# bing164/PL-VI-ORBSLAM3

Measured on AMD Instinct MI355X. Metric: frames/sec ORB+LSD extract+match, 640×480 mono, 1/2/4/8 MI355X, higher is better.
Workload: dtype u8; 1 GPU; C1+C2+C3: ORB extract (1000 feats, 1.2, 8 levels, FAST 20/7) || LSD+LBD (200 lines, scale 0.8, 2 octaves) as one HIP-stream schedule, then ORB kNN-2 + LineMatcher::match vs previous frame; batch=3072, width=640, height=480, parallelism=sequence-sharded x1, gather=False, inflight=2

## Files before the change

pl-vi-orbslam3_amd/csrc/lines_kernels.hpp:

```cpp
#include <hip/hip_runtime.h>

#include "block_prims.h"
#include "lines_device.h"
#include "plvi_common.h"
#include "plvi_math.h"
#include "std_sort.h"

namespace plvi {

constexpr double kNotdef = -1024.0;
constexpr float kNotdefF = -1024.0f;
constexpr double kD2R = 3.14159265358979323846 / 180;
constexpr double kPi = 3.14159265358979323846;
constexpr double kLog10Of11 = 0x1.0a98b6050c56fp+0;

__global__ __launch_bounds__(256) void lsd_half_kernel(const uint8_t* __restrict__ src, size_t s_frame, size_t s_row,
                                                       uint8_t* __restrict__ dst, int dw, int dh, size_t d_frame) {
    const int f = blockIdx.y;
    const int i = blockIdx.x * 256 + threadIdx.x;
    if (i >= dw * dh) return;
    const int y = i / dw, x = i % dw;
    const uint8_t* S0 = src + (size_t)f * s_frame + (size_t)(2 * y) * s_row;
    const uint8_t* S1 = S0 + s_row;
    const int s = S0[2 * x] + S0[2 * x + 1] + S1[2 * x] + S1[2 * x + 1];
// ... 1113 lines not shown
        const int D0 = sd - su, D1 = sd1 - su1;
        const int pk = S1 | (D1 + 1024) << 12, pkl = S0 | (D0 + 1024) << 12;
        const int L = dpp_from_left(pk);
        const int R = dpp_from_right(pkl);
        const int Sl = xl ? S1 : (L & 4095), Dl = xl ? D1 : (L >> 12) - 1024;
        const int Sr = xr ? S0 : (R & 4095), Dr = xr ? D0 : (R >> 12) - 1024;
        const bool last0 = xa + 1 >= w;
        const int Sr0 = last0 ? Sl : S1, Dr0 = last0 ? Dl : D1;
        const int gx0 = Sr0 - Sl, gy0 = Dl + 2 * D0 + Dr0;
        const int gx1 = Sr - S0, gy1 = D0 + 2 * D1 + Dr;
        short2* o = Gp + (size_t)y * w + xa;
        if (out0) o[0] = make_short2((short)gx0, (short)gy0);
        if (out1) o[1] = make_short2((short)gx1, (short)gy1);
    };
    uint32_t pv[8];
#pragma unroll
    for (int k = 0; k < 8; ++k) pv[k] = load_row(k - 2);
    const int rend = 2 * h + 3;
    for (int rb = -2; rb < rend - 2; rb += 8) {
#pragma unroll
        for (int k = 0; k < 8; ++k) {
            const int r = rb + k;
            if (r > 2 * h) break;
            const uint32_t V = pv[k];
            if (r + 8 <= 2 * h) pv[k] = load_row(r + 8);
#pragma unroll
            for (int q = 0; q < 4; ++q) {
                pe[q] = pe[q + 1];
                po[q] = po[q + 1];
            }
            pe[4] = V & 0x00ff00ffu;
            po[4] = (V >> 8) & 0x00ff00ffu;
            if ((k & 1) || r < 2) continue;
            const int y = (r - 2) >> 1;
            const uint32_t Ve = pe[0] + pe[4] + 4 * (pe[1] + pe[3]) + 6 * pe[2];
            const uint32_t Vo = po[0] + po[4] + 4 * (po[1] + po[3]) + 6 * po[2];
            const uint32_t Vel = (uint32_t)dpp_from_left((int)Ve), Vol = (uint32_t)dpp_from_left((int)Vo);
            const uint32_t Ver = (uint32_t)dpp_from_right((int)Ve);
            const uint32_t s0 = (Vel >> 16) + 4 * (Vol >> 16) + 6 * (Ve & 0xffffu) + 4 * (Vo & 0xffffu) + (Ve >> 16);
            const uint32_t s1 = (Ve & 0xffffu) + 4 * (Vo & 0xffffu) + 6 * (Ve >> 16) + 4 * (Vo >> 16) + (Ver & 0xffffu);
            const int P = (int)((s0 + 128u) >> 8) | (int)((s1 + 128u) >> 8) << 8;
            if (y == 1) sobel_row(0, P, p0, P);
            else if (y >= 2) sobel_row(y - 1, pm1, p0, P);
            pm1 = p0;
            p0 = P;
        }
    }
    if (h >= 2) sobel_row(h - 1, pm1, p0, pm1);
    else sobel_row(0, p0, p0, p0);
}

__constant__ float c_gaussG[63];
__constant__ float c_gaussL[21];
__constant__ unsigned char c_comb[64];

__global__ __launch_bounds__(64) void lbd_describe_kernel(const LineOctDev* __restrict__ octs,
                                                          const short2* __restrict__ g_all,
                                                          const plvi_keyline* __restrict__ kls,
                                                          const int* __restrict__ counts, int fcap,
                                                          uint8_t* __restrict__ desc) {
    __shared__ float rq[8][64];
    __shared__ float bs[72];
    __shared__ float dv[72];
    const int li = blockIdx.x, f = blockIdx.y;
    if (li >= counts[f]) return;
    const plvi_keyline kl = kls[(size_t)f * fcap + li];
    const LineOctDev& od = octs[kl.octave];
    const short2* pg = g_all + od.loff + (size_t)f * od.lplane;
    const short realWidth = (short)od.lw;
    const short imageWidth = realWidth - 1;
    const short imageHeight = (short)(od.lh - 1);
    const short lengthOfLSP = (short)kl.numOfPixels;
    const short halfWidth = (lengthOfLSP - 1) / 2;
    const short halfHeight = (63 - 1) / 2;
    const float mX = (float)(0.5 * (double)(kl.sPointInOctaveX + kl.ePointInOctaveX));
    const float mY = (float)(0.5 * (double)(kl.sPointInOctaveY + kl.ePointInOctaveY));
    const float dL0 = plvi_cosf(kl.angle), dL1 = plvi_sinf(kl.angle);
    const float dO0 = -dL1, dO1 = dL0;
    const int h = threadIdx.x;
    float pL = 0, nL = 0, pO = 0, nO = 0;
    __shared__ int sidx[64][9];
    auto& sg = sidx;
    {
        float sX = -dL0 * halfWidth + dL1 * halfHeight + mX;
        float sY = -dL1 * halfWidth - dL0 * halfHeight + mY;
        for (int k = 0; k < h; ++k) {
            sX -= dL1;
            sY += dL0;
        }
        const int* pgi = reinterpret_cast<const int*>(pg);
        const int kk = h & 7, rr = h >> 3;
        for (int w0 = 0; w0 < lengthOfLSP; w0 += 8) {
#pragma unroll
            for (int k = 0; k < 8; ++k) {
                short t = (short)__builtin_roundf(sX);
                const short xc = (t < 0) ? 0 : (t > imageWidth) ? imageWidth : t;
                t = (short)__builtin_roundf(sY);
                const short yc = (t < 0) ? 0 : (t > imageHeight) ? imageHeight : t;
                sidx[h][k] = yc * realWidth + xc;
                sX += dL0;
                sY += dL1;
            }
            __builtin_amdgcn_wave_barrier();
            __builtin_amdgcn_fence(__ATOMIC_ACQ_REL, "wavefront");
            int gv[8];
            const bool okk = w0 + kk < lengthOfLSP;
#pragma unroll
            for (int i = 0; i < 8; ++i) {
                const int r = 8 * i + rr;
                gv[i] = (r < 63 && okk) ? pgi[sidx[r][kk]] : 0;
            }
#pragma unroll
            for (int i = 0; i < 8; ++i) sg[8 * i + rr][kk] = gv[i];
            __builtin_amdgcn_wave_barrier();
            __builtin_amdgcn_fence(__ATOMIC_ACQ_REL, "wavefront");
            if (h < 63) {
#pragma unroll
                for (int k = 0; k < 8; ++k) {
                    if (w0 + k >= lengthOfLSP) break;
                    const short2 g = __builtin_bit_cast(short2, sg[h][k]);
                    const short dx = g.x, dy = g.y;
                    const float gDL = dx * dL0 + dy * dL1;
                    const float gDO = dx * dO0 + dy * dO1;
                    if (gDL > 0) pL += gDL;
                    else nL -= gDL;
                    if (gDO > 0) pO += gDO;
                    else nO -= gDO;
                }
            }
            __builtin_amdgcn_wave_barrier();
            __builtin_amdgcn_fence(__ATOMIC_ACQ_REL, "wavefront");
        }
    }
    if (h < 63) {
        const float c = c_gaussG[h];
        const float pLr = c * pL, nLr = c * nL, pOr = c * pO, nOr = c * nO;
        rq[0][h] = pLr; rq[1][h] = nLr; rq[2][h] = pLr * pLr; rq[3][h] = nLr * nLr;
        rq[4][h] = pOr; rq[5][h] = nOr; rq[6][h] = pOr * pOr; rq[7][h] = nOr * nOr;
    }
    __syncthreads();
    for (int a = h; a < 72; a += 64) {
        const int b = a >> 3, q = a & 7;
        const bool sq = (q & 2) != 0;
        float acc = 0.f;
        const int r0 = max(0, 7 * (b - 1)), r1 = min(62, 7 * (b + 2) - 1);
        for (int r = r0; r <= r1; ++r) {
            const int j = r / 7, m = r - 7 * j;
            const float c = j == b ? c_gaussL[m + 7] : j == b + 1 ? c_gaussL[m + 14] : c_gaussL[m];
            const float x = rq[q][r];
            acc += sq ? c * c * x : c * x;
        }
        bs[a] = acc;
    }
    __syncthreads();
    if (h < 36) {
        const int b = h >> 2, k = h & 3;
        const int qs = (k < 2 ? 0 : 4) + (k & 1);
        const float invN = (b == 0 || b == 8) ? (float)(1.0 / (7 * 2.0)) : (float)(1.0 / (7 * 3.0));
        const float t = bs[8 * b + qs] * invN;
        dv[8 * b + k] = t;
        dv[8 * b + 4 + k] = __builtin_sqrtf(bs[8 * b + qs + 2] * invN - t * t);
    }
    __syncthreads();
    __shared__ float s_t[3];
    if (h == 0) {
        float tM = 0, tS = 0;
        for (int b = 0; b < 9; ++b) {
            const float* v = dv + 8 * b;
            tM += v[0] * v[0]; tM += v[1] * v[1]; tM += v[2] * v[2]; tM += v[3] * v[3];
            tS += v[4] * v[4]; tS += v[5] * v[5]; tS += v[6] * v[6]; tS += v[7] * v[7];
        }
        s_t[0] = 1 / __builtin_sqrtf(tM);
        s_t[1] = 1 / __builtin_sqrtf(tS);
    }
    __syncthreads();
    for (int i = h; i < 72; i += 64) {
        float v = dv[i] * ((i & 7) < 4 ? s_t[0] : s_t[1]);
        if ((double)v > 0.4) v = (float)0.4;
        dv[i] = v;
    }
    __syncthreads();
    if (h == 0) {
        float t = 0;
        for (int i = 0; i < 72; ++i) t += dv[i] * dv[i];
        s_t[2] = 1 / __builtin_sqrtf(t);
    }
    __syncthreads();
    for (int i = h; i < 72; i += 64) dv[i] = dv[i] * s_t[2];
    __syncthreads();
    if (h < 32) {
        const float* f1 = dv + 8 * c_comb[2 * h];
        const float* f2 = dv + 8 * c_comb[2 * h + 1];
        unsigned r = 0;
        for (int i = 0; i < 8; ++i)
            if (f1[i] > f2[i]) r += 1u << i;
        desc[((size_t)f * fcap + li) * 32 + h] = (uint8_t)r;
    }
}

}
```

pl-vi-orbslam3_amd/csrc/lines_pipeline.hip:

```cpp
#include <hip/hip_runtime.h>

#include <algorithm>
#include <cmath>
#include <cstdlib>
#include <cstring>
#include <memory>
#include <vector>

#include "lines_device.h"
#include "lines_kernels.hpp"
#include "lsd_grow_mw.hpp"
#include "plvi_common.h"

extern "C" int plvi_orb_internal_blur_event(plvi_orb_extractor* h, hipEvent_t ev);
extern "C" int plvi_orb_internal_stage_event(plvi_orb_extractor* h, int stage, hipEvent_t ev);

namespace plvi {

static inline int lround_h(float v) { return (int)lrintf(v); }
static inline int lround_h(double v) { return (int)lrint(v); }
static inline int lfloor_h(float v) { int i = (int)v; return i - (i > v); }

static double cv_exp64f(double x) {
    const double a0s = .9670371139572337719125840413672004409288e-2;
// ... 12 lines not shown
}

static void gauss_kernel_f64(int n, double sigma, double* k, bool cvExp) {
    const double scale2X = -0.125 / (sigma * sigma);
    const int n2 = (n - 1) / 2;
    std::vector<double> values(n2 + 1);
    double sum = 0;
    for (int i = 0, x = 1 - n; i < n2; ++i, x += 2) {
        const double a = (double)(x * x) * scale2X;
        double t = cvExp ? cv_exp64f(a) : std::exp(a);
        values[i] = t;
        sum += t;
    }
    sum *= 2;
    sum += 1.0;
    const double mul1 = 1.0 / sum;
    for (int i = 0; i < n2; ++i) k[i] = k[n - 1 - i] = values[i] * mul1;
    k[n2] = 1.0 * mul1;
}

struct LinePipeline {
    plvi_line_params prm{};
    int W = 0, H = 0, Bcap = 0, device = 0, nOct = 0, fcap = 0;
    hipStream_t stream = nullptr;
    hipStream_t aux[2] = {nullptr, nullptr};
    hipEvent_t evSobelGo = nullptr;
    hipEvent_t evFork = nullptr, evPrep = nullptr, evSobel = nullptr, evOrb = nullptr, evCrit = nullptr,
               evBlur = nullptr, evGate = nullptr, evGrow2 = nullptr, evPair = nullptr;
    bool growAfterBlur = true, sobelWithGrow = false, growSplit = false;
    int sobelGate = -1;
    bool sobelAfterGrow = false;
    hipStream_t critStream = nullptr;
    hipStream_t crit2 = nullptr;
    hipStream_t octStream = nullptr;
    int orbAfterPrep = 1;
    std::vector<LineOctDev> oct;
    std::vector<float> scaleF, invScaleF;
    double SCALE = 0.8, prec = 0, rho = 0, min_length = 0;
    double gk[7]{};
    int lbdTaps[3] = {14, 62, 104};
    DevBuf d_oct, d_tabs, octImg, pix, modg, seedcs, gbits, qspill, regs, regpts, rawLines, nlines, klTmp, klOut, fnOut, cntOut, descOut, lbdBlur,
        lbdG, err, staging, mwOwn, mwSlot, mwGrow, sortPos;
    size_t qspillFrame = 0, gbitsFrame = 0, lbdPlaneTotal = 0;
    int lastFrames = 0;
    static constexpr int kStages = 5, kRing = 512;
    bool prof = false;
    int profRuns = 0;
    std::vector<hipEvent_t> evs;

    static constexpr int kKRing = 4096;
    bool ktime = false;
    int kn = 0;
    std::vector<hipEvent_t> kev;
    std::vector<hipEvent_t> kevS[3];
    int knS[3] = {0, 0, 0};
    int ktiming(int on) {
        if (on && kev.empty()) {
            kev.resize(2 * kKRing);
            for (auto& e : kev) PLVI_CHECK(hipEventCreate(&e));
            for (auto& v : kevS) {
                v.resize(2 * kKRing);
                for (auto& e : v) PLVI_CHECK(hipEventCreate(&e));
            }
        }
        ktime = on != 0;
        if (on) kn = knS[0] = knS[1] = knS[2] = 0;
        return PLVI_OK;
    }
    void ktimeS(int k, int edge, hipStream_t st) {
        if (!ktime || knS[k] >= kKRing) return;
        (void)hipEventRecord(kevS[k][2 * knS[k] + edge], st);
        if (edge) ++knS[k];
    }
    int ktiming_read_kind(int kind, float* total_ms, int* launches) {
        if (kind == 0) return ktiming_read(total_ms, launches);
        if (kind < 1 || kind > 3) return PLVI_E_BADARG;
        const int k = kind - 1;
        float tot = 0.f;
        for (int i = 0; i < knS[k]; ++i) {
            PLVI_CHECK(hipEventSynchronize(kevS[k][2 * i + 1]));
            float t = 0.f;
            PLVI_CHECK(hipEventElapsedTime(&t, kevS[k][2 * i], kevS[k][2 * i + 1]));
            tot += t;
        }
        if (total_ms) *total_ms = tot;
        if (launches) *launches = knS[k];
        return PLVI_OK;
    }
    int ktiming_read(float* total_ms, int* launches) {
        float tot = 0.f;
        for (int i = 0; i < kn; ++i) {
            PLVI_CHECK(hipEventSynchronize(kev[2 * i + 1]));
            float t = 0.f;
            PLVI_CHECK(hipEventElapsedTime(&t, kev[2 * i], kev[2 * i + 1]));
            tot += t;
        }
        if (total_ms) *total_ms = tot;
        if (launches) *launches = kn;
        return PLVI_OK;
    }

    ~LinePipeline() {
        for (auto e : kev) (void)hipEventDestroy(e);
        for (auto& v : kevS)
            for (auto e : v) (void)hipEventDestroy(e);
        for (auto e : evs) (void)hipEventDestroy(e);
        for (auto e : {evFork, evPrep, evSobel, evOrb, evCrit, evBlur, evGate, evGrow2, evPair, evSobelGo})
            if (e) (void)hipEventDestroy(e);
        if (critStream) (void)hipStreamDestroy(critStream);
        if (crit2) (void)hipStreamDestroy(crit2);
        if (octStream) (void)hipStreamDestroy(octStream);
        for (auto a : aux)
            if (a) (void)hipStreamDestroy(a);
        if (stream) (void)hipStreamDestroy(stream);
    }

    int init(const plvi_line_params* p, int width, int height, int max_batch, int dev) {
        if (!p || width <= 0 || height <= 0 || max_batch <= 0) return PLVI_E_BADARG;
        if (p->refine != 0 || p->extractor != 0) return PLVI_E_BADARG;
        if (p->nlevels <= 0 || p->nlevels > kLineMaxOct || p->nfeatures < 0) return PLVI_E_BADARG;
        prm = *p;
        W = width; H = height; Bcap = max_batch; device = dev; nOct = p->nlevels;
        PLVI_CHECK(hipSetDevice(device));
        PLVI_CHECK(hipStreamCreateWithFlags(&stream, hipStreamNonBlocking));
        {
            int least = 0, greatest = 0;
            PLVI_CHECK(hipDeviceGetStreamPriorityRange(&least, &greatest));
            const char* e1 = getenv("PLVI_STREAM_PRIO");
            const bool prio = !e1 || atoi(e1) != 0;
// ... 100 lines not shown
                    yb[2 * dy + 1] = fy;
                }
                d.xmax = xmax;
                std::vector<int> strips;
                for (int X0 = 0; X0 < d.sw;) {
                    const int gx0 = xofs[X0];
                    int E = X0;
                    while (E < d.sw && xofs[E] + (E < xmax ? 1 : 0) - gx0 + 3 <= 60) ++E;
                    const int X1 = E == d.sw ? E : E - 1;
                    if (X1 <= X0) return PLVI_E_BADARG;
                    strips.insert(strips.end(), {X0, X1, gx0, E - X0});
                    X0 = X1;
                }
                for (int dy = 0; dy < d.sh; ++dy) {
                    const int r1 = yrow[2 * dy + 1], r0 = yrow[2 * dy];
                    if (r0 > r1 || r1 - r0 > 1 || (dy > 0 && r1 < yrow[2 * dy - 1])) return PLVI_E_BADARG;
                }
                d.nstrips = (int)strips.size() / 4;
                d.tabStrips = put(strips.data(), strips.size() * 4);
                for (int nb : {1, kPrepBands}) {
                    std::vector<int> bands;
                    for (int b = 0; b < nb; ++b) {
                        const int dyA = (int)((long long)d.sh * b / nb), dyB = (int)((long long)d.sh * (b + 1) / nb);
                        bands.insert(bands.end(), {dyA, dyB, dyA == 0 ? -3 : yrow[2 * dyA] - 3, 0});
                    }
                    (nb == 1 ? d.tabBands1 : d.tabBandsK) = put(bands.data(), bands.size() * 4);
                }
                d.tabXofs = put(xofs.data(), xofs.size() * 4);
                d.tabXa = put(xa.data(), xa.size() * 4);
                d.tabYrow = put(yrow.data(), yrow.size() * 4);
                d.tabYb = put(yb.data(), yb.size() * 4);
            }
            d.lw = l == 0 ? W : oct[l - 1].lw / 2;
            d.lh = l == 0 ? H : oct[l - 1].lh / 2;
            d.lplane = (long long)d.lw * d.lh;
            d.loff = (long long)lOff;
            lOff += (size_t)d.lplane * Bcap;
        }
        lbdPlaneTotal = lOff;
        qspillFrame = (maxSplane + 1) & ~size_t(1);
        for (auto& d : oct) gbitsFrame = std::max(gbitsFrame, (size_t)d.sh * (size_t)((d.sw + 31) / 32));
        if (d_oct.alloc(sizeof(LineOctDev) * nOct) || d_tabs.alloc(tabs.size())) return PLVI_E_HIP;
        PLVI_CHECK(hipMemcpy(d_oct.p, oct.data(), sizeof(LineOctDev) * nOct, hipMemcpyHostToDevice));
        PLVI_CHECK(hipMemcpy(d_tabs.p, tabs.data(), tabs.size(), hipMemcpyHostToDevice));
        {
            float gL[21], gG[63];
            double u = (7 * 3 - 1) / 2, sg = (7 * 2 + 1) / 2, inv = -1 / (2 * sg * sg);
            for (int i = 0; i < 21; ++i) { double dis = i - u; gL[i] = (float)std::exp(dis * dis * inv); }
            u = (9 * 7 - 1) / 2; sg = u; inv = -1 / (2 * sg * sg);
            for (int i = 0; i < 63; ++i) { double dis = i - u; gG[i] = (float)std::exp(dis * dis * inv); }
            static const unsigned char comb[64] = {0, 1, 0, 2, 0, 3, 0, 4, 0, 5, 0, 6, 1, 2, 1, 3, 1, 4, 1, 5, 1, 6,
                                                   2, 3, 2, 4, 2, 5, 2, 6, 2, 7, 2, 8, 3, 4, 3, 5, 3, 6, 3, 7, 3, 8,
                                                   4, 5, 4, 6, 4, 7, 4, 8, 5, 6, 5, 7, 5, 8, 6, 7, 6, 8, 7, 8};
            PLVI_CHECK(hipMemcpyToSymbol(HIP_SYMBOL(c_gaussL), gL, sizeof(gL)));
            PLVI_CHECK(hipMemcpyToSymbol(HIP_SYMBOL(c_gaussG), gG, sizeof(gG)));
            PLVI_CHECK(hipMemcpyToSymbol(HIP_SYMBOL(c_comb), comb, sizeof(comb)));
        }
        if (octImg.alloc(std::max<size_t>(imgOff, 16)) || pix.alloc(sizeof(float) * sOff) ||
            modg.alloc(sizeof(double) * sOff) || seedcs.alloc(sizeof(float2) * sOff) ||
            gbits.alloc(sizeof(unsigned) * gbitsFrame * nOct * Bcap) || qspill.alloc(sizeof(unsigned) * qspillFrame * nOct * Bcap) ||
            rawLines.alloc(sizeof(LsdLine) * (size_t)kLsdRawCap * nOct * Bcap) ||
            regs.alloc(sizeof(LsdRegion) * (size_t)kLsdRawCap * nOct * Bcap) ||
            regpts.alloc(sizeof(unsigned) * qspillFrame * nOct * Bcap) ||
            nlines.alloc(sizeof(int) * nOct * Bcap) || klTmp.alloc(sizeof(plvi_keyline) * (size_t)kKlCap * Bcap) ||
            sortPos.alloc(sizeof(unsigned short) * 2 * (size_t)kKlCap * Bcap) ||
            klOut.alloc(sizeof(plvi_keyline) * (size_t)fcap * Bcap) || fnOut.alloc(sizeof(double) * 3 * fcap * Bcap) ||
            cntOut.alloc(sizeof(int) * Bcap) || descOut.alloc((size_t)32 * fcap * Bcap) ||
            lbdBlur.alloc((size_t)W * H * Bcap) || lbdG.alloc(sizeof(short2) * lbdPlaneTotal) ||
            err.alloc(sizeof(int) * Bcap) || staging.alloc((size_t)W * H))
            return PLVI_E_HIP;
        PLVI_CHECK(hipMemset(err.p, 0, sizeof(int) * Bcap));
        size_t maxSw = 0;
        for (auto& d : oct) maxSw = std::max(maxSw, (size_t)d.sw);
        const size_t wprMax = (maxSw + 31) / 32;
        size_t budget = 6 * 1024;
        if (const char* e = getenv("PLVI_GROW_LDS")) budget = (size_t)atol(e);
        budget = std::min<size_t>(budget, 160 * 1024);
        growRB = 64;
        if (const char* e = getenv("PLVI_GROW_RB")) growRB = atoi(e);
        if (growRB < 2 || (growRB & (growRB - 1)) || growRB > 1024) return PLVI_E_BADARG;
        growQL = budget >= 32 * 1024 ? 1024 : 256;
        const size_t fixed = (size_t)growQL * sizeof(unsigned) + (size_t)growRB * wprMax * sizeof(unsigned);
        const size_t perRow = maxSw * sizeof(float);
        growR = 0;
        if (fixed + perRow * 2 <= budget) {
            growR = 2;
            while (growR * 2 <= 1024 && fixed + perRow * growR * 2 <= budget) growR *= 2;
        }
        if (const char* e = getenv("PLVI_GROW_RD")) growR = atoi(e);
        if (growR < 0 || (growR & (growR - 1)) || growR == 1 || growR > 1024) return PLVI_E_BADARG;
        growSmem = (fixed + perRow * growR + 15) & ~size_t(15);
        if (growSmem > 160 * 1024) return PLVI_E_BADARG;
        growWPW = (int)std::max<size_t>(1, std::min<size_t>(kGrowWaves, (160 * 1024) / growSmem));
        for (const void* k : {(const void*)lsd_grow_kernel<false, false>, (const void*)lsd_grow_kernel<true, false>,
                              (const void*)lsd_grow_kernel<false, true>, (const void*)lsd_grow_kernel<true, true>,
                              (const void*)lsd_grow_kernel<false, true, true>})
            PLVI_CHECK(hipFuncSetAttribute(k, hipFuncAttributeMaxDynamicSharedMemorySize, (int)(growSmem * growWPW)));
        mwMaxFrames = 256;
        if (const char* e = getenv("PLVI_GROW_MW")) mwMaxFrames = atoi(e);
        if (const char* e = getenv("PLVI_GROW_TPW")) growTPW = std::max(0, atoi(e));
        mwMaxFrames = std::min(mwMaxFrames, Bcap);
        if (mwMaxFrames > 0) {
            const size_t nwords = gbitsFrame;
            const size_t fixedMw = sizeof(MwCtl) + 8 * kMwLog +
                                   4 * (3 * nwords + (size_t)kMwWaves * kMwRB * wprMax + (size_t)kMwWaves * kMwGQ);
            const size_t ldsMax = 160 * 1024;
            mwSlots = fixedMw < ldsMax ? (int)std::min<size_t>(kMwMaxSlots, (ldsMax - fixedMw) / kMwSlotBytes) : 0;
// ... 117 lines not shown
                           (const float2*)seedcs.as<float2>(), gbits.as<unsigned>(), gbitsFrame,
                           qspill.as<unsigned>(), qspillFrame, prec, regs.as<LsdRegion>(), regpts.as<unsigned>(),
                           qspillFrame, nlines.as<int>(), err.as<int>(), growR, growRB, growQL, nOct, oBase, oCount,
                           growStats, nf, (int)growSmem, growWPW);
    }
    void launch_rect(int nf, int oBase, int oCount, hipStream_t st) {
        const int bx = nf <= 16 ? 8 : nf < kRectLargeNf ? kRectLaneBlocks : kRectLaneBlocksLarge;
        auto rectK = nf <= kRectSmallNf ? lsd_rect_lanes_kernel<kRectUSmall> : lsd_rect_lanes_kernel<kRectU>;
        ktimeS(2, 0, st);
        hipLaunchKernelGGL(rectK, dim3(bx, nf, oCount), dim3(256), 0, st, d_oct.as<LineOctDev>(),
                           (const double*)modg.as<double>(), (const LsdRegion*)regs.as<LsdRegion>(),
                           (const unsigned*)regpts.as<unsigned>(), qspillFrame, (const int*)nlines.as<int>(), prec,
                           SCALE, rawLines.as<LsdLine>(), oBase, nOct, qspill.as<double>(), qspillFrame / 2,
                           (int)(qspillFrame / 2));
        ktimeS(2, 1, st);
    }
    void launch_grow_assemble(int nf, hipStream_t st, bool grown = false, bool rect0 = false) {
        if (!grown) launch_grow(nf, 0, nOct, st);
        launch_rect(nf, 0, rect0 ? 1 : nOct, st);
        mark(3, st);
        hipLaunchKernelGGL(line_assemble_kernel, dim3(nf), dim3(256), 0, st, d_oct.as<LineOctDev>(), nOct,
                           (const LsdLine*)rawLines.as<LsdLine>(), (const int*)nlines.as<int>(), min_length,
                           prm.nfeatures, fcap, klOut.as<plvi_keyline>(), fnOut.as<double>(), cntOut.as<int>(),
                           klTmp.as<plvi_keyline>(), err.as<int>(), sortPos.as<unsigned short>());
        mark(4, st);
    }

    int launch_sobel(const uint8_t* d_frames, int nf, size_t frame_stride, size_t row_stride, hipStream_t st) {
        const LineOctDev& d0 = oct[0];
        {
            const int ns = (d0.lw + 4 * kLbOutLanes - 1) / (4 * kLbOutLanes);
            const int sw4 = ((d0.lw + ns - 1) / ns + 3) & ~3;
            ktimeS(0, 0, st);
            hipLaunchKernelGGL(lbd_sobel0_kernel, dim3((d0.lw + sw4 - 1) / sw4, nf, kLbBands), dim3(64), 0, st, d_frames,
                               frame_stride, row_stride, d0.lw, d0.lh, sw4, lbdBlur.as<uint8_t>(),
                               lbdG.as<short2>() + d0.loff, (size_t)d0.lplane, lbdTaps[0], lbdTaps[1], lbdTaps[2]);
            ktimeS(0, 1, st);
        }
        for (int l = 1; l < nOct; ++l) {
            const LineOctDev& d = oct[l];
            if (l > 1) return PLVI_E_BADARG;
            const int ns = (d.lw + 2 * kLb2OutLanes - 1) / (2 * kLb2OutLanes);
            const int sw2 = ((d.lw + ns - 1) / ns + 1) & ~1;
            ktimeS(1, 0, st);
            hipLaunchKernelGGL(lbd_sobel1_kernel, dim3((d.lw + sw2 - 1) / sw2, nf), dim3(64), 0, st,
                               (const uint8_t*)lbdBlur.as<uint8_t>(), d0.lw, d0.lh, (size_t)d0.lplane, d.lw, d.lh,
                               sw2, lbdG.as<short2>() + d.loff, (size_t)d.lplane);
            ktimeS(1, 1, st);
        }
        return PLVI_OK;
    }

    void launch_describe(int nf, hipStream_t st) {
        hipLaunchKernelGGL(lbd_describe_kernel, dim3(fcap, nf), dim3(64), 0, st, d_oct.as<LineOctDev>(),
                           (const short2*)lbdG.as<short2>(),
                           (const plvi_keyline*)klOut.as<plvi_keyline>(), (const int*)cntOut.as<int>(), fcap,
                           descOut.as<uint8_t>());
        mark(5, st);
    }

    int run(const uint8_t* d_frames, int nf, size_t frame_stride, size_t row_stride, hipStream_t st) {
        if (nf <= 0 || nf > Bcap) return PLVI_E_BADARG;
        if (!st) st = stream;
        lastFrames = nf;
        hipStreamCaptureStatus cs = hipStreamCaptureStatusNone;
        PLVI_CHECK(hipStreamIsCapturing(st, &cs));
        const bool fork = !prof && aux[1] && cs == hipStreamCaptureStatusNone;
        int rc = PLVI_OK;
        if (fork) {
            PLVI_CHECK(hipEventRecord(evFork, st));
            PLVI_CHECK(hipStreamWaitEvent(aux[1], evFork, 0));
            rc = launch_sobel(d_frames, nf, frame_stride, row_stride, aux[1]);
            PLVI_CHECK(hipEventRecord(evSobel, aux[1]));
        }
        mark(0, st);
        if (fork && nOct > 1 && nf <= mwMaxFrames) {
            launch_prep(d_frames, nf, frame_stride, row_stride, st, 0, 1);
            PLVI_CHECK(hipEventRecord(evPrep, st));
            PLVI_CHECK(hipStreamWaitEvent(aux[0], evPrep, 0));
            launch_prep(d_frames, nf, frame_stride, row_stride, aux[0], 1, nOct);
            launch_grow(nf, 1, nOct - 1, aux[0]);
            launch_rect(nf, 1, nOct - 1, aux[0]);
            PLVI_CHECK(hipEventRecord(evGrow2, aux[0]));
            launch_grow(nf, 0, 1, st);
            PLVI_CHECK(hipStreamWaitEvent(st, evGrow2, 0));
            launch_grow_assemble(nf, st, true, true);
        } else {
            launch_prep(d_frames, nf, frame_stride, row_stride, st);
            launch_grow_assemble(nf, st);
        }
        if (fork) {
            PLVI_CHECK(hipStreamWaitEvent(st, evSobel, 0));
        } else {
            rc = launch_sobel(d_frames, nf, frame_stride, row_stride, st);
        }
        if (rc) return rc;
        launch_describe(nf, st);
        if (prof && profRuns < kRing) ++profRuns;
        PLVI_CHECK(hipGetLastError());
        return PLVI_OK;
    }

    struct StepMatch {
        int *idx0, *d0, *idx1, *d1;
        float nnr;
        int *lscratch, *lm12, *lnm;
    };
    int run_with_orb(const uint8_t* d_frames, int nf, size_t frame_stride, size_t row_stride, hipStream_t st,
                     plvi_orb_extractor* orb, int lap0, int lap1, const StepMatch* sm = nullptr) {
        if (nf <= 0 || nf > Bcap) return PLVI_E_BADARG;
// ... 371 lines not shown
```

pl-vi-orbslam3_amd/csrc/plvi_math.h:

```cpp
#pragma once
#include <stdint.h>
#include <string.h>

#ifdef __HIPCC__
#define PLVI_HD __host__ __device__ __forceinline__
#else
#define PLVI_HD static inline
#endif

namespace plvi {

PLVI_HD uint32_t f2u(float f) { uint32_t u; memcpy(&u, &f, 4); return u; }
PLVI_HD float u2f(uint32_t u) { float f; memcpy(&f, &u, 4); return f; }
PLVI_HD uint64_t d2u(double d) { uint64_t u; memcpy(&u, &d, 8); return u; }
PLVI_HD double u2d(uint64_t u) { double d; memcpy(&d, &u, 8); return d; }
PLVI_HD double fmad(double a, double b, double c) { return __builtin_fma(a, b, c); }

PLVI_HD double rfma(double a, double b, double c) { return __builtin_fma(a, b, c); }
PLVI_HD float rfmaf(float a, float b, float c) { return __builtin_fmaf(a, b, c); }

struct SinCosF {
    double c0, c1, s1, c2, s2, c3, s3, c4;
};
#define PLVI_HPI_INV 0x1.45f306dc9c883p+23
// ... 72 lines not shown
        uint32_t xi = f2u(y);
        int sign = xi >> 31;
        x = reduce_large(xi, &n);
        int q = (n + sign) & 3;
        double s = (q == 1 || q == 2) ? -1.0 : 1.0;
        return sinf_poly(x * s, x * x, sincosf_tab(((n + sign) & 2) ? 1 : 0), n);
    }
    return (y - y) / (y - y);
}

PLVI_HD float plvi_cosf(float y) {
    double x = y;
    int n;
    if (abstop12(y) < abstop12(0x1.921fb6p-1f)) {
        double x2 = x * x;
        if (abstop12(y) < abstop12(0x1p-12f)) return 1.0f;
        return sinf_poly(x, x2, sincosf_tab(0), 1);
    } else if (abstop12(y) < abstop12(120.0f)) {
        x = reduce_fast(x, &n);
        double s = (n & 3) == 1 || (n & 3) == 2 ? -1.0 : 1.0;
        return sinf_poly(x * s, x * x, sincosf_tab((n & 2) ? 1 : 0), n ^ 1);
    } else if (abstop12(y) < abstop12(__builtin_inff())) {
        uint32_t xi = f2u(y);
        int sign = xi >> 31;
        x = reduce_large(xi, &n);
        int q = (n + sign) & 3;
        double s = (q == 1 || q == 2) ? -1.0 : 1.0;
        return sinf_poly(x * s, x * x, sincosf_tab(((n + sign) & 2) ? 1 : 0), n ^ 1);
    }
    return (y - y) / (y - y);
}

PLVI_HD void plvi_sincosf_pos(float y, float* sp, float* cp) {
    int n;
    const double x = reduce_fast((double)y, &n);
    const double sg = (n & 3) == 1 || (n & 3) == 2 ? -1.0 : 1.0;
    const double neg = (n & 2) ? -1.0 : 1.0;
    const double xs = x * sg, x2 = x * x;
    const double x3 = xs * x2;
    const double s1 = fmad(x2, -0x1.994eb3774cf24p-13, 0x1.1107605230bc4p-7);
    const double x7 = x3 * x2;
    const double sv = fmad(x3, -0x1.555545995a603p-3, xs);
    const float S = (float)fmad(x7, s1, sv);
    const double x4 = x2 * x2;
    const double c2 = fmad(x2, neg * 0x1.99343027bf8c3p-16, neg * -0x1.6c087e89a359dp-10);
    const double c1 = fmad(x2, neg * -0x1.ffffffd0c621cp-2, neg * 0x1.0p+0);
    const double x6 = x4 * x2;
    const double cv = fmad(x4, neg * 0x1.55553e1068f19p-5, c1);
    const float C = (float)fmad(x6, c2, cv);
    float s = (n & 1) ? C : S, c = (n & 1) ? S : C;
    if (abstop12(y) < abstop12(0x1p-12f)) { s = y; c = 1.0f; }
    *sp = s;
    *cp = c;
}

PLVI_HD float plvi_fast_atan2(float y, float x) {
    const float k = (float)(180 / 3.1415926535897932384626433832795);
    const float p1 = 0.9997878412794807f * k, p3 = -0.3258083974640975f * k;
    const float p5 = 0.1555786518463281f * k, p7 = -0.04432655554792128f * k;
    const float eps = (float)2.2204460492503131e-16;
    float ax = __builtin_fabsf(x), ay = __builtin_fabsf(y);
    const bool ge = ax >= ay;
    const float c = (ge ? ay : ax) / ((ge ? ax : ay) + eps);
    const float c2 = c * c;
    const float pc = (((p7 * c2 + p5) * c2 + p3) * c2 + p1) * c;
    float a = ge ? pc : 90.f - pc;
    if (x < 0) a = 180.f - a;
    if (y < 0) a = 360.f - a;
    return a;
}

PLVI_HD float plvi_atanf_core(float x) {
    const float atanhi[4] = {4.6364760399e-01f, 7.8539812565e-01f, 9.8279368877e-01f, 1.5707962513e+00f};
    const float atanlo[4] = {5.0121582440e-09f, 3.7748947079e-08f, 3.4473217170e-08f, 7.5497894159e-08f};
    const float aT[11] = {3.3333334327e-01f,  -2.0000000298e-01f, 1.4285714924e-01f, -1.1111110449e-01f,
                          9.0908870101e-02f,  -7.6918758452e-02f, 6.6610731184e-02f, -5.8335702866e-02f,
                          4.9768779427e-02f,  -3.6531571299e-02f, 1.6285819933e-02f};
    float w, s1, s2, z;
    int32_t ix, hx, id;
    hx = (int32_t)f2u(x);
    ix = hx & 0x7fffffff;
    if (ix >= 0x4c000000) {
        if (ix > 0x7f800000) return x + x;
        if (hx > 0) return atanhi[3] + atanlo[3];
        return -atanhi[3] - atanlo[3];
    }
    if (ix < 0x3ee00000) {
        if (ix < 0x31000000) return x;
        id = -1;
    } else {
        x = __builtin_fabsf(x);
        if (ix < 0x3f980000) {
            if (ix < 0x3f300000) { id = 0; x = ((float)2.0 * x - 1.0f) / ((float)2.0 + x); }
            else { id = 1; x = (x - 1.0f) / (x + 1.0f); }
        } else {
            if (ix < 0x401c0000) { id = 2; x = (x - (float)1.5) / (1.0f + (float)1.5 * x); }
            else { id = 3; x = -(float)1.0 / x; }
        }
    }
    z = x * x;
    w = z * z;
    s1 = z * (aT[0] + w * (aT[2] + w * (aT[4] + w * (aT[6] + w * (aT[8] + w * aT[10])))));
    s2 = w * (aT[1] + w * (aT[3] + w * (aT[5] + w * (aT[7] + w * aT[9]))));
    if (id < 0) return x - x * (s1 + s2);
    z = atanhi[id] - ((x * (s1 + s2) - atanlo[id]) - x);
    return (hx < 0) ? -z : z;
// ... 253 lines not shown
```

Before: 61180 frames/s.

## Restructure LBD describe kernel into multi-wave persistent blocks with wave-level reductions

The LBD descriptor kernel now runs four independent waves per block. Each wave loops over several keylines with a grid stride and prefetches the next keyline record into lanes. Per-lane sample start positions come from a DPP lane-shift scan instead of a per-thread serial loop. Gradients are gathered in 16-wide chunks through a padded LDS tile, and the band sums and the three normalisation passes use readlane coefficients and vectorised LDS reads across the wave, replacing single-thread serial loops and block barriers. This adds a precomputed squared-Gaussian table and per-kernel timing events, and relies on wave-synchronous LDS reuse being correct.

```diff
diff --git a/pl-vi-orbslam3_amd/csrc/lines_kernels.hpp b/pl-vi-orbslam3_amd/csrc/lines_kernels.hpp
--- a/pl-vi-orbslam3_amd/csrc/lines_kernels.hpp
+++ b/pl-vi-orbslam3_amd/csrc/lines_kernels.hpp
@@ -1189,150 +1189,207 @@
 
 __constant__ float c_gaussG[63];
 __constant__ float c_gaussL[21];
+__constant__ float c_gaussLL[21];
 __constant__ unsigned char c_comb[64];
 
-__global__ __launch_bounds__(64) void lbd_describe_kernel(const LineOctDev* __restrict__ octs,
-                                                          const short2* __restrict__ g_all,
-                                                          const plvi_keyline* __restrict__ kls,
-                                                          const int* __restrict__ counts, int fcap,
-                                                          uint8_t* __restrict__ desc) {
-    __shared__ float rq[8][64];
-    __shared__ float bs[72];
-    __shared__ float dv[72];
-    const int li = blockIdx.x, f = blockIdx.y;
-    if (li >= counts[f]) return;
-    const plvi_keyline kl = kls[(size_t)f * fcap + li];
-    const LineOctDev& od = octs[kl.octave];
-    const short2* pg = g_all + od.loff + (size_t)f * od.lplane;
-    const short realWidth = (short)od.lw;
-    const short imageWidth = realWidth - 1;
-    const short imageHeight = (short)(od.lh - 1);
-    const short lengthOfLSP = (short)kl.numOfPixels;
-    const short halfWidth = (lengthOfLSP - 1) / 2;
-    const short halfHeight = (63 - 1) / 2;
-    const float mX = (float)(0.5 * (double)(kl.sPointInOctaveX + kl.ePointInOctaveX));
-    const float mY = (float)(0.5 * (double)(kl.sPointInOctaveY + kl.ePointInOctaveY));
-    const float dL0 = plvi_cosf(kl.angle), dL1 = plvi_sinf(kl.angle);
-    const float dO0 = -dL1, dO1 = dL0;
-    const int h = threadIdx.x;
-    float pL = 0, nL = 0, pO = 0, nO = 0;
-    __shared__ int sidx[64][9];
-    auto& sg = sidx;
-    {
+constexpr int kLbdWaves = 4;
+constexpr int kLbdLinesPerWave = 4;
+constexpr int kLbdSlotsPerLine = 65536;
+constexpr int kLbdChunk = 16;
+constexpr int kLbdTileStride = kLbdChunk + 1;
+constexpr int kLbdBandRows = 7 + 63 + 7;
+
+struct LbdWaveLds {
+    union {
+        int tile[64 * kLbdTileStride];
+        float rq[kLbdBandRows * 8];
+    };
+    alignas(16) float dv[72];
+    alignas(16) float sq[72];
+};
+static_assert(sizeof(plvi_keyline) == 17 * sizeof(int), "keyline record: one dword per lane 0..16");
+static_assert(kLbdBandRows * 8 <= 64 * kLbdTileStride, "row sums alias the sample tile");
+
+__device__ __forceinline__ void lbd_wave_sync() {
+    __builtin_amdgcn_wave_barrier();
+    __builtin_amdgcn_fence(__ATOMIC_ACQ_REL, "wavefront");
+}
+
+__device__ __forceinline__ float lbd_from_lane_below(float own, float next) {
+    return __builtin_bit_cast(float, __builtin_amdgcn_update_dpp(__builtin_bit_cast(int, own), __builtin_bit_cast(int, next),
+                                                                 0x138, 0xf, 0xf, false));
+}
+
+__global__ __launch_bounds__(64 * kLbdWaves) __attribute__((amdgpu_waves_per_eu(8, 8))) void lbd_describe_kernel(
+    const LineOctDev* __restrict__ octs, int nOct, const short2* __restrict__ g_all, const plvi_keyline* __restrict__ kls,
+    const int* __restrict__ counts, int fcap, uint8_t* __restrict__ desc) {
+    __shared__ LbdWaveLds lds[kLbdWaves];
+    const int wv = __builtin_amdgcn_readfirstlane((int)(threadIdx.x >> 6));
+    const int h = threadIdx.x & 63;
+    const int f = blockIdx.y;
+    const int cnt = min(counts[f], fcap);
+    const int stride = gridDim.x * kLbdWaves;
+    int li = blockIdx.x * kLbdWaves + wv;
+    if (li >= cnt) return;
+    LbdWaveLds& L = lds[wv];
+    const float cG = c_gaussG[min(h, 62)];
+    const int cLv = __builtin_bit_cast(int, c_gaussL[min(h, 20)]), cLLv = __builtin_bit_cast(int, c_gaussLL[min(h, 20)]);
+    const int combA = 8 * c_comb[(2 * h) & 63], combB = 8 * c_comb[(2 * h + 1) & 63];
+    const LineOctDev& o0 = octs[0];
+    const LineOctDev& o1 = octs[nOct > 1 ? 1 : 0];
+    const int lw0 = o0.lw, lh0 = o0.lh, lw1 = o1.lw, lh1 = o1.lh;
+    const long long loff0 = o0.loff, lpl0 = o0.lplane, loff1 = o1.loff, lpl1 = o1.lplane;
+    const int* recs = reinterpret_cast<const int*>(kls + (size_t)f * fcap);
+    const unsigned recLane = h < 17 ? h : 0;
+    int rec = recs[(unsigned)li * 17u + recLane];
+    const int bb = h >> 2, bk = h & 3;
+    const int bqs = (bk < 2 ? 0 : 4) + (bk & 1);
+    const float invN = (bb == 0 || bb == 8) ? (float)(1.0 / (7 * 2.0)) : (float)(1.0 / (7 * 3.0));
+    const int kk = h & 7, rr = h >> 3;
+    for (;;) {
+        const float angle = __builtin_bit_cast(float, __builtin_amdgcn_readlane(rec, 0));
+        const int octave = __builtin_amdgcn_readlane(rec, 2);
+        const float sPX = __builtin_bit_cast(float, __builtin_amdgcn_readlane(rec, 11));
+        const float sPY = __builtin_bit_cast(float, __builtin_amdgcn_readlane(rec, 12));
+        const float ePX = __builtin_bit_cast(float, __builtin_amdgcn_readlane(rec, 13));
+        const float ePY = __builtin_bit_cast(float, __builtin_amdgcn_readlane(rec, 14));
+        const int numOfPixels = __builtin_amdgcn_readlane(rec, 16);
+        const int liNext = li + stride;
+        rec = recs[(unsigned)min(liNext, fcap - 1) * 17u + recLane];
+        const bool oc1 = octave != 0;
+        const char* pgb = reinterpret_cast<const char*>(g_all + (oc1 ? loff1 : loff0) + (size_t)f * (oc1 ? lpl1 : lpl0));
+        const short realWidth = (short)(oc1 ? lw1 : lw0);
+        const short imageWidth = realWidth - 1;
+        const short imageHeight = (short)((oc1 ? lh1 : lh0) - 1);
+        const short lengthOfLSP = (short)numOfPixels;
+        const short halfWidth = (lengthOfLSP - 1) / 2;
+        const short halfHeight = (63 - 1) / 2;
+        const float mX = (float)(0.5 * (double)(sPX + ePX));
+        const float mY = (float)(0.5 * (double)(sPY + ePY));
+        const float dL0 = plvi_cosf(angle), dL1 = plvi_sinf(angle);
+        const float dO0 = -dL1, dO1 = dL0;
+        float pL = 0, nL = 0, pO = 0, nO = 0;
         float sX = -dL0 * halfWidth + dL1 * halfHeight + mX;
         float sY = -dL1 * halfWidth - dL0 * halfHeight + mY;
-        for (int k = 0; k < h; ++k) {
-            sX -= dL1;
-            sY += dL0;
-        }
-        const int* pgi = reinterpret_cast<const int*>(pg);
-        const int kk = h & 7, rr = h >> 3;
-        for (int w0 = 0; w0 < lengthOfLSP; w0 += 8) {
-#pragma unroll
-            for (int k = 0; k < 8; ++k) {
-                short t = (short)__builtin_roundf(sX);
-                const short xc = (t < 0) ? 0 : (t > imageWidth) ? imageWidth : t;
-                t = (short)__builtin_roundf(sY);
-                const short yc = (t < 0) ? 0 : (t > imageHeight) ? imageHeight : t;
-                sidx[h][k] = yc * realWidth + xc;
+#pragma unroll
+        for (int k = 0; k < 62; ++k) {
+            sX = lbd_from_lane_below(sX, sX - dL1);
+            sY = lbd_from_lane_below(sY, sY + dL0);
+        }
+        int* trow = L.tile + h * kLbdTileStride;
+        for (int w0 = 0; w0 < lengthOfLSP; w0 += kLbdChunk) {
+#pragma unroll
+            for (int k = 0; k < kLbdChunk; ++k) {
+                const int xc = plvi_round_clamp_i16(sX, imageWidth);
+                const int yc = plvi_round_clamp_i16(sY, imageHeight);
+                trow[k] = (yc * realWidth + xc) * 4;
                 sX += dL0;
                 sY += dL1;
-            }
-            __builtin_amdgcn_wave_barrier();
-            __builtin_amdgcn_fence(__ATOMIC_ACQ_REL, "wavefront");
-            int gv[8];
-            const bool okk = w0 + kk < lengthOfLSP;
-#pragma unroll
-            for (int i = 0; i < 8; ++i) {
-                const int r = 8 * i + rr;
-                gv[i] = (r < 63 && okk) ? pgi[sidx[r][kk]] : 0;
-            }
-#pragma unroll
-            for (int i = 0; i < 8; ++i) sg[8 * i + rr][kk] = gv[i];
-            __builtin_amdgcn_wave_barrier();
-            __builtin_amdgcn_fence(__ATOMIC_ACQ_REL, "wavefront");
-            if (h < 63) {
-#pragma unroll
-                for (int k = 0; k < 8; ++k) {
-                    if (w0 + k >= lengthOfLSP) break;
-                    const short2 g = __builtin_bit_cast(short2, sg[h][k]);
-                    const short dx = g.x, dy = g.y;
-                    const float gDL = dx * dL0 + dy * dL1;
-                    const float gDO = dx * dO0 + dy * dO1;
-                    if (gDL > 0) pL += gDL;
-                    else nL -= gDL;
-                    if (gDO > 0) pO += gDO;
-                    else nO -= gDO;
-                }
-            }
-            __builtin_amdgcn_wave_barrier();
-            __builtin_amdgcn_fence(__ATOMIC_ACQ_REL, "wavefront");
-        }
-    }
-    if (h < 63) {
-        const float c = c_gaussG[h];
-        const float pLr = c * pL, nLr = c * nL, pOr = c * pO, nOr = c * nO;
-        rq[0][h] = pLr; rq[1][h] = nLr; rq[2][h] = pLr * pLr; rq[3][h] = nLr * nLr;
-        rq[4][h] = pOr; rq[5][h] = nOr; rq[6][h] = pOr * pOr; rq[7][h] = nOr * nOr;
-    }
-    __syncthreads();
-    for (int a = h; a < 72; a += 64) {
-        const int b = a >> 3, q = a & 7;
-        const bool sq = (q & 2) != 0;
-        float acc = 0.f;
-        const int r0 = max(0, 7 * (b - 1)), r1 = min(62, 7 * (b + 2) - 1);
-        for (int r = r0; r <= r1; ++r) {
-            const int j = r / 7, m = r - 7 * j;
-            const float c = j == b ? c_gaussL[m + 7] : j == b + 1 ? c_gaussL[m + 14] : c_gaussL[m];
-            const float x = rq[q][r];
-            acc += sq ? c * c * x : c * x;
-        }
-        bs[a] = acc;
-    }
-    __syncthreads();
-    if (h < 36) {
-        const int b = h >> 2, k = h & 3;
-        const int qs = (k < 2 ? 0 : 4) + (k & 1);
-        const float invN = (b == 0 || b == 8) ? (float)(1.0 / (7 * 2.0)) : (float)(1.0 / (7 * 3.0));
-        const float t = bs[8 * b + qs] * invN;
-        dv[8 * b + k] = t;
-        dv[8 * b + 4 + k] = __builtin_sqrtf(bs[8 * b + qs + 2] * invN - t * t);
-    }
-    __syncthreads();
-    __shared__ float s_t[3];
-    if (h == 0) {
+                if ((k & 3) == 3) __builtin_amdgcn_sched_barrier(0);
+            }
+            lbd_wave_sync();
+            int gv[2 * 8];
+#pragma unroll
+            for (int i = 0; i < 2 * 8; ++i) {
+                const int r = 8 * (i >> 1) + rr, k = kk + 8 * (i & 1);
+                gv[i] = *reinterpret_cast<const int*>(pgb + (unsigned)L.tile[r * kLbdTileStride + k]);
+            }
+            const bool ok0 = w0 + kk < lengthOfLSP, ok1 = w0 + kk + 8 < lengthOfLSP;
+#pragma unroll
+            for (int i = 0; i < 2 * 8; ++i) {
+                const int r = 8 * (i >> 1) + rr, k = kk + 8 * (i & 1);
+                L.tile[r * kLbdTileStride + k] = ((i & 1) ? ok1 : ok0) ? gv[i] : 0;
+            }
+            lbd_wave_sync();
+#pragma unroll
+            for (int k = 0; k < kLbdChunk; ++k) {
+                const short2 g = __builtin_bit_cast(short2, trow[k]);
+                const short dx = g.x, dy = g.y;
+                const float gDL = dx * dL0 + dy * dL1;
+                const float gDO = dx * dO0 + dy * dO1;
+                pL += __builtin_fmaxf(gDL, 0.f);
+                nL += __builtin_fmaxf(-gDL, 0.f);
+                pO += __builtin_fmaxf(gDO, 0.f);
+                nO += __builtin_fmaxf(-gDO, 0.f);
+                if ((k & 3) == 3) __builtin_amdgcn_sched_barrier(0);
+            }
+            lbd_wave_sync();
+        }
+        if (h < 56) {
+            L.rq[h] = 0.f;
+            L.rq[(63 + 7) * 8 + h] = 0.f;
+        }
+        if (h < 63) {
+            const float pLr = cG * pL, nLr = cG * nL, pOr = cG * pO, nOr = cG * nO;
+            float4* q = reinterpret_cast<float4*>(L.rq + (h + 7) * 8);
+            q[0] = make_float4(pLr, nLr, pLr * pLr, nLr * nLr);
+            q[1] = make_float4(pOr, nOr, pOr * pOr, nOr * nOr);
+        }
+        lbd_wave_sync();
+        float m, sd;
+        {
+            float accL = 0.f, accS = 0.f;
+            const float* x = L.rq + 56 * bb + bqs;
+#pragma unroll
+            for (int t = 0; t < 21; ++t) {
+                const float c = __builtin_bit_cast(float, __builtin_amdgcn_readlane(cLv, t));
+                const float cc = __builtin_bit_cast(float, __builtin_amdgcn_readlane(cLLv, t));
+                accL += c * x[8 * t];
+                accS += cc * x[8 * t + 2];
+            }
+            m = accL * invN;
+            sd = __builtin_sqrtf(accS * invN - m * m);
+        }
+        const int im = 8 * bb + bk, is = im + 4;
+        lbd_wave_sync();
+        if (h < 36) {
+            L.sq[im] = m * m;
+            L.sq[is] = sd * sd;
+        }
+        lbd_wave_sync();
         float tM = 0, tS = 0;
+#pragma unroll
         for (int b = 0; b < 9; ++b) {
-            const float* v = dv + 8 * b;
-            tM += v[0] * v[0]; tM += v[1] * v[1]; tM += v[2] * v[2]; tM += v[3] * v[3];
-            tS += v[4] * v[4]; tS += v[5] * v[5]; tS += v[6] * v[6]; tS += v[7] * v[7];
-        }
-        s_t[0] = 1 / __builtin_sqrtf(tM);
-        s_t[1] = 1 / __builtin_sqrtf(tS);
-    }
-    __syncthreads();
-    for (int i = h; i < 72; i += 64) {
-        float v = dv[i] * ((i & 7) < 4 ? s_t[0] : s_t[1]);
-        if ((double)v > 0.4) v = (float)0.4;
-        dv[i] = v;
-    }
-    __syncthreads();
-    if (h == 0) {
+            const float4 vm = *reinterpret_cast<const float4*>(L.sq + 8 * b);
+            const float4 vs = *reinterpret_cast<const float4*>(L.sq + 8 * b + 4);
+            tM += vm.x; tM += vm.y; tM += vm.z; tM += vm.w;
+            tS += vs.x; tS += vs.y; tS += vs.z; tS += vs.w;
+        }
+        m = m * (1 / __builtin_sqrtf(tM));
+        sd = sd * (1 / __builtin_sqrtf(tS));
+        if ((double)m > 0.4) m = (float)0.4;
+        if ((double)sd > 0.4) sd = (float)0.4;
+        lbd_wave_sync();
+        if (h < 36) {
+            L.sq[im] = m * m;
+            L.sq[is] = sd * sd;
+        }
+        lbd_wave_sync();
         float t = 0;
-        for (int i = 0; i < 72; ++i) t += dv[i] * dv[i];
-        s_t[2] = 1 / __builtin_sqrtf(t);
-    }
-    __syncthreads();
-    for (int i = h; i < 72; i += 64) dv[i] = dv[i] * s_t[2];
-    __syncthreads();
-    if (h < 32) {
-        const float* f1 = dv + 8 * c_comb[2 * h];
-        const float* f2 = dv + 8 * c_comb[2 * h + 1];
-        unsigned r = 0;
-        for (int i = 0; i < 8; ++i)
-            if (f1[i] > f2[i]) r += 1u << i;
-        desc[((size_t)f * fcap + li) * 32 + h] = (uint8_t)r;
-    }
-}
-
-}
+#pragma unroll
+        for (int i = 0; i < 72; i += 4) {
+            const float4 v = *reinterpret_cast<const float4*>(L.sq + i);
+            t += v.x; t += v.y; t += v.z; t += v.w;
+        }
+        const float s2 = 1 / __builtin_sqrtf(t);
+        if (h < 36) {
+            L.dv[im] = m * s2;
+            L.dv[is] = sd * s2;
+        }
+        lbd_wave_sync();
+        if (h < 32) {
+            const float* f1 = L.dv + combA;
+            const float* f2 = L.dv + combB;
+            unsigned r = 0;
+#pragma unroll
+            for (int i = 0; i < 8; ++i)
+                if (f1[i] > f2[i]) r += 1u << i;
+            (desc + ((size_t)f * fcap + li) * 32)[(unsigned)h] = (uint8_t)r;
+        }
+        li = liNext;
+        if (li >= cnt) break;
+        lbd_wave_sync();
+    }
+}
+
+}
diff --git a/pl-vi-orbslam3_amd/csrc/lines_pipeline.hip b/pl-vi-orbslam3_amd/csrc/lines_pipeline.hip
--- a/pl-vi-orbslam3_amd/csrc/lines_pipeline.hip
+++ b/pl-vi-orbslam3_amd/csrc/lines_pipeline.hip
@@ -88,8 +88,8 @@
     bool ktime = false;
     int kn = 0;
     std::vector<hipEvent_t> kev;
-    std::vector<hipEvent_t> kevS[3];
-    int knS[3] = {0, 0, 0};
+    std::vector<hipEvent_t> kevS[4];
+    int knS[4] = {0, 0, 0, 0};
     int ktiming(int on) {
         if (on && kev.empty()) {
             kev.resize(2 * kKRing);
@@ -100,7 +100,7 @@
             }
         }
         ktime = on != 0;
-        if (on) kn = knS[0] = knS[1] = knS[2] = 0;
+        if (on) kn = knS[0] = knS[1] = knS[2] = knS[3] = 0;
         return PLVI_OK;
     }
     void ktimeS(int k, int edge, hipStream_t st) {
@@ -110,7 +110,7 @@
     }
     int ktiming_read_kind(int kind, float* total_ms, int* launches) {
         if (kind == 0) return ktiming_read(total_ms, launches);
-        if (kind < 1 || kind > 3) return PLVI_E_BADARG;
+        if (kind < 1 || kind > 4) return PLVI_E_BADARG;
         const int k = kind - 1;
         float tot = 0.f;
         for (int i = 0; i < knS[k]; ++i) {
@@ -317,7 +317,10 @@
             static const unsigned char comb[64] = {0, 1, 0, 2, 0, 3, 0, 4, 0, 5, 0, 6, 1, 2, 1, 3, 1, 4, 1, 5, 1, 6,
                                                    2, 3, 2, 4, 2, 5, 2, 6, 2, 7, 2, 8, 3, 4, 3, 5, 3, 6, 3, 7, 3, 8,
                                                    4, 5, 4, 6, 4, 7, 4, 8, 5, 6, 5, 7, 5, 8, 6, 7, 6, 8, 7, 8};
+            float gLL[21];
+            for (int i = 0; i < 21; ++i) gLL[i] = gL[i] * gL[i];
             PLVI_CHECK(hipMemcpyToSymbol(HIP_SYMBOL(c_gaussL), gL, sizeof(gL)));
+            PLVI_CHECK(hipMemcpyToSymbol(HIP_SYMBOL(c_gaussLL), gLL, sizeof(gLL)));
             PLVI_CHECK(hipMemcpyToSymbol(HIP_SYMBOL(c_gaussG), gG, sizeof(gG)));
             PLVI_CHECK(hipMemcpyToSymbol(HIP_SYMBOL(c_comb), comb, sizeof(comb)));
         }
@@ -541,10 +544,15 @@
     }
 
     void launch_describe(int nf, hipStream_t st) {
-        hipLaunchKernelGGL(lbd_describe_kernel, dim3(fcap, nf), dim3(64), 0, st, d_oct.as<LineOctDev>(),
+        const long long slots = (long long)fcap * nf;
+        const int per = (int)std::min<long long>(kLbdLinesPerWave, std::max<long long>(1, slots / kLbdSlotsPerLine));
+        const int gx = ((fcap + per - 1) / per + kLbdWaves - 1) / kLbdWaves;
+        ktimeS(3, 0, st);
+        hipLaunchKernelGGL(lbd_describe_kernel, dim3(gx, nf), dim3(64 * kLbdWaves), 0, st, d_oct.as<LineOctDev>(), nOct,
                            (const short2*)lbdG.as<short2>(),
                            (const plvi_keyline*)klOut.as<plvi_keyline>(), (const int*)cntOut.as<int>(), fcap,
                            descOut.as<uint8_t>());
+        ktimeS(3, 1, st);
         mark(5, st);
     }
 
diff --git a/pl-vi-orbslam3_amd/csrc/plvi_math.h b/pl-vi-orbslam3_amd/csrc/plvi_math.h
--- a/pl-vi-orbslam3_amd/csrc/plvi_math.h
+++ b/pl-vi-orbslam3_amd/csrc/plvi_math.h
@@ -148,6 +148,14 @@
     if (abstop12(y) < abstop12(0x1p-12f)) { s = y; c = 1.0f; }
     *sp = s;
     *cp = c;
+}
+
+PLVI_HD int plvi_round_clamp_i16(float v, int hi) {
+    const float t = __builtin_truncf(v);
+    int i = (int)t;
+    i += (v - t >= 0.5f) ? 1 : 0;
+    i = (short)i;
+    return i < 0 ? 0 : i > hi ? hi : i;
 }
 
 PLVI_HD float plvi_fast_atan2(float y, float x) {
```

New measurement: 62410 frames/s (median of 6 runs). +2.0%, better.
